# LinXueyuanStdio/LaTeX_OCR

Measured on NVIDIA H100. Metric: formula-images/sec (train step, 128x512 px, seq<=150), higher is better.
Workload: dtype bf16

## Files before the change

### latex_ocr_b200/csrc/lo_common.cuh

```cuda
#pragma once
#include <cuda_runtime.h>
#include <cuda_bf16.h>
#include <stdint.h>
#include <stdio.h>
#include <string.h>

#include "../../include/latex_ocr_b200.h"

typedef __nv_bfloat16 bf16;

namespace lo {

extern char g_err[512];
extern int64_t g_launches;

inline int fail(int code, const char* fmt, const char* a = "", long b = 0, long c = 0) {
  snprintf(g_err, sizeof(g_err), fmt, a, b, c);
  return code;
}

#define LO_CHECK_ARG(cond, what)                                                        \
  do {                                                                                  \
    if (!(cond)) return lo::fail(LO_EINVAL, "%s: invalid argument: " what " (line %ld)", __func__, __LINE__); \
  } while (0)
// ... 189 lines not shown
int gemm_nn(const void* A, int dtA, int64_t lda, const void* B, int dtB, int64_t ldb, void* C, int dtC, int64_t ldc,
            int M, int N, int K, int accumulate, int impl, cudaStream_t st);
int colsum(const void* X, int dt, float* out, int M, int N, int64_t ld, int accumulate, cudaStream_t st);

struct AttFwdArgs {
  const void *att1, *enc;
  const float* att2; int64_t att2_stride;
  const float* wf;
  float* alpha; int64_t alpha_stride;
  float* ctx; float* gate_pre; int64_t gate_stride; float* gctx; bf16* gctx_bf;
  int B, R;
  void* work;
  int rows_per_img;
  int act;
  int a_ch;
  uint8_t* mask_out;
  int abi = 0;
};
struct AttBwdArgs {
  const void *att1, *enc;
  const float *att2, *gate; int64_t o1_stride;
  const float* wf; const float* alpha; int64_t alpha_stride;
  const float* ctx; const float* dgctx; int64_t dg_stride;
  const float* dreg; int64_t dreg_stride; const float* sreg; int64_t sreg_stride;
  float* de; float* datt2; float* dgp; int64_t dcat_stride; bf16* datt2_bf; bf16* dgp_bf; float* dctx_out;
  int B, R;
  void* work;
  float* dwf_part;
  int act;
  int a_ch;
  const uint8_t* mask_in;
  int abi = 0;
  void* datt1 = nullptr;
  int ordered_dwf = 0;
};
int attention_fwd_pipe(const AttFwdArgs& x, int dt, int C, cudaStream_t st);
int attention_bwd_pipe(const AttBwdArgs& x, int dt, int C, cudaStream_t st);
inline int64_t att_partials_offset(int B) { return B <= 1024 ? 4096 : ((int64_t)B * 4 + 255) / 256 * 256; }
struct AttRagged {
  const int32_t* reg_off;
  const int32_t* reg_off_host;
  void* map;
  int ctas;
};
int64_t attention_ragged_map_bytes(int B);
int attention_ragged_prepare(AttRagged& rg, int B, int rpi, cudaStream_t st);
int attention_fwd_ragged(const AttFwdArgs& x, const AttRagged& rg, int dt, int C, cudaStream_t st);

bool tc_available();
int tc_gemm_nt(const bf16* A, int64_t lda, const bf16* W, int64_t ldw, void* C, int dtC, int64_t ldc,
               int M, int N, int K, const float* bias, int accumulate, int relu, cudaStream_t st);
int tc_gemm_nt_ex(const bf16* A, int64_t lda, const bf16* W, int64_t ldw, void* C, int dtC, int64_t ldc, int M, int N, int K,
                  const float* bias, int accumulate, int relu, int splits, int atomic_acc, int small_n_tile, cudaStream_t st);
int skinny_gemm_nt(const bf16* A, int64_t lda, const bf16* W, int64_t ldw, float* C, int64_t ldc, int M, int N, int K, const float* bias,
                   int splits, int atomic_acc, cudaStream_t st);
int resident_ctas(const void* kernel, int threads, size_t smem);
int tc_gemm_tn(const bf16* A, int64_t lda, const bf16* B, int64_t ldb, float* C, int64_t ldc, int M, int N, int K, cudaStream_t st);
int tc_gemm_tn_batched(const bf16* A, int64_t sAk, int64_t sAb, const bf16* B, int64_t sBk, int64_t sBb, float* C, int64_t ldc,
                       int64_t sCb, int M, int N, int K, int batch, cudaStream_t st);
int tc_conv3x3_wgrad(const bf16* x, const bf16* dy, float* dw, int N, int H, int W, int Cin, int Cout, int pad, cudaStream_t st);
int tc_conv3x3(const bf16* x, const bf16* w, const float* bias, const bf16* mask, bf16* y,
               int N, int H, int W, int Cin, int Cout, int pad, int relu, cudaStream_t st);

}
```

### latex_ocr_b200/csrc/lo_decoder.cu

```cuda
#include "lo_common.cuh"
#include "lo_ptx.cuh"

namespace lo {

#define LO_ATT_THREADS 256
#define LO_ATT_WARPS 8
#define LO_ATT_MAXSPLIT 16

static inline int att_splits(int B) {
  int s = (444 + B - 1) / B;
  if (s < 1) s = 1;
  if (s > LO_ATT_MAXSPLIT) s = LO_ATT_MAXSPLIT;
  return s;
}

__device__ __forceinline__ float ldcg_f(const float* p) { return __ldcg(p); }

template <typename T, int NV>
__global__ void __launch_bounds__(LO_ATT_THREADS) attention_fwd_kernel(
    const T* __restrict__ att1, const T* __restrict__ enc, const float* __restrict__ att2, int64_t att2_stride,
    const float* __restrict__ wf, float* __restrict__ alpha, int64_t alpha_stride, float* __restrict__ ctx,
    float* __restrict__ gate_pre, int64_t gate_stride, float* __restrict__ gctx, bf16* __restrict__ gctx_bf, int R, int nsplit,
    int* __restrict__ counters, float* __restrict__ partials, int rpi) {
  constexpr int CH = NV * 256;
// ... 1112 lines not shown

__global__ void split_bf16_kernel(const float* __restrict__ x, bf16* __restrict__ hi, bf16* __restrict__ lo, int64_t n) {
  for (int64_t i = blockIdx.x * (int64_t)blockDim.x + threadIdx.x; i < n; i += (int64_t)gridDim.x * blockDim.x) {
    const float v = x[i];
    const bf16 h = __float2bfloat16_rn(v);
    hi[i] = h;
    lo[i] = __float2bfloat16_rn(v - __bfloat162float(h));
  }
}

static int forward_prologue(const lo_decoder_args* a, const Dims& d, cudaStream_t st) {
  const int dt = a->dt;
  const int rpi = a->rows_per_img > 1 ? a->rows_per_img : 1;
  const int enc_rows = a->reg_off_host ? a->reg_off_host[d.B / rpi] : (d.B / rpi) * d.R;
  LO_TRY(gemm_nt(a->enc, dt, d.C, a->w_enc_att, dt, d.C, a->att1, dt, d.A, enc_rows, d.A, d.C, a->b_enc_att, 0, 0, a->impl, st));
  const BfViews bv0 = bf_views(a, d);
  if (bv0.on && d.E % 64 == 0) {
    LO_TRY(tc_gemm_nt_ex((const bf16*)a->emb, d.E, (const bf16*)a->w_ih, d.E + d.C, a->ptab, LO_F32, d.G, d.V, d.G, d.E, a->b_ih, 0, 0, 1,
                         0, 0, st));
  } else {
    LO_TRY(gemm_nt(a->emb, dt, d.E, a->w_ih, dt, d.E + d.C, a->ptab, LO_F32, d.G, d.V, d.G, d.E, a->b_ih, 0, 0, LO_IMPL_SIMT, st));
  }
  {
    dim3 grid(cdiv(d.C, 256), d.B);
    if (a->reg_off)
      LO_DISPATCH_DT(dt, T, (mean_segments_kernel<T><<<grid, 256, 0, st>>>((const T*)a->enc, a->mean, a->reg_off, d.C, rpi)));
    else
      LO_DISPATCH_DT(dt, T, (mean_rows_kernel<T><<<grid, 256, 0, st>>>((const T*)a->enc, a->mean, d.R, d.C, rpi)));
    LO_LAUNCH_OK();
  }
  const size_t es = dt == LO_F32 ? 4 : 2;
  if (bv0.on && d.C % 64 == 0 && d.T >= 2) {
    bf16* mean_hi = bv0.gctx;
    bf16* mean_lo = bv0.gctx + (int64_t)d.B * d.C;
    split_bf16_kernel<<<cdiv((long)d.B * d.C, 256), 256, 0, st>>>(a->mean, mean_hi, mean_lo, (int64_t)d.B * d.C);
    LO_LAUNCH_OK();
    const bf16* w_h = (const bf16*)a->w_init;
    const bf16* w_c = w_h + (int64_t)d.D * d.C;
    LO_TRY(tc_gemm_nt_ex(mean_hi, d.C, w_h, d.C, a->hall, LO_F32, d.D, d.B, d.D, d.C, a->b_init, 0, 0, 1, 0, 1, st));
    LO_TRY(tc_gemm_nt_ex(mean_lo, d.C, w_h, d.C, a->hall, LO_F32, d.D, d.B, d.D, d.C, nullptr, 1, 0, 1, 0, 1, st));
    LO_TRY(tc_gemm_nt_ex(mean_hi, d.C, w_c, d.C, a->call, LO_F32, d.D, d.B, d.D, d.C, a->b_init + d.D, 0, 0, 1, 0, 1, st));
    LO_TRY(tc_gemm_nt_ex(mean_lo, d.C, w_c, d.C, a->call, LO_F32, d.D, d.B, d.D, d.C, nullptr, 1, 0, 1, 0, 1, st));
  } else {
    LO_TRY(gemm_nt(a->mean, LO_F32, d.C, a->w_init, dt, d.C, a->hall, LO_F32, d.D, d.B, d.D, d.C, a->b_init, 0, 0, LO_IMPL_SIMT, st));
    LO_TRY(gemm_nt(a->mean, LO_F32, d.C, (const char*)a->w_init + (size_t)d.D * d.C * es, dt, d.C, a->call, LO_F32, d.D, d.B,
                   d.D, d.C, a->b_init + d.D, 0, 0, LO_IMPL_SIMT, st));
  }
  const BfViews bv = bf_views(a, d);
  if (bv.on) LO_TRY(lo_cast(a->hall, LO_F32, bv.hall, LO_BF16, (int64_t)d.B * d.D, (void*)st));
  return LO_OK;
}

static int step_gemm_nt(bool tc, const float* A32, const bf16* Abf, int64_t lda, const void* W, int dtW, int64_t ldw, float* C,
                        int64_t ldc, int M, int N, int K, const float* bias, int acc, int splits, int atomic_acc, cudaStream_t st) {
  if (tc && g_opt_skinny_mma && M <= 64) return skinny_gemm_nt(Abf, lda, (const bf16*)W, ldw, C, ldc, M, N, K, bias, splits, atomic_acc, st);
  if (tc)
    return tc_gemm_nt_ex(Abf, lda, (const bf16*)W, ldw, C, LO_F32, ldc, M, N, K, bias, 0, 0, g_opt_det ? 1 : splits, atomic_acc, 1, st);
  return gemm_nt(A32, LO_F32, lda, W, dtW, ldw, C, LO_F32, ldc, M, N, K, bias, acc, 0, LO_IMPL_SIMT, st);
}

static int head_nt(const lo_decoder_args* a, bool tc, const float* h32, const bf16* hbf, int64_t ldh, float* logits, int64_t ldl, int M,
                   cudaStream_t st) {
  if (tc) return gemm_nt(hbf, LO_BF16, ldh, a->w_fc, LO_BF16, a->D, logits, LO_F32, ldl, M, a->V, a->D, a->b_fc, 0, 0, LO_IMPL_TC, st);
  return gemm_nt(h32, LO_F32, ldh, a->w_fc, a->dt, a->D, logits, LO_F32, ldl, M, a->V, a->D, a->b_fc, 0, 0, LO_IMPL_SIMT, st);
}

static int forward_step(const lo_decoder_args* a, const Dims& d, int t, int nrows, const AttRagged* rg, const int64_t* tok,
                        int64_t tok_stride, float* hd_t, int64_t hd_stride, const float* dmask_t, cudaStream_t st) {
  const int dt = a->dt;
  const bool sampling = a->ss_prob && hd_t;
  const size_t es = dt == LO_F32 ? 4 : 2;
  const int64_t cur = (int64_t)t * d.B, nxt = (int64_t)(t + 1) * d.B;
  float* o1 = a->out1 + cur * d.O1;
  const BfViews bv = bf_views(a, d);
  if (!(g_opt_dbg_skip & 4))
    LO_TRY(step_gemm_nt(bv.on, a->hall + cur * d.D, bv.on ? bv.hall + cur * d.D : nullptr, d.D, a->wcat1, dt, d.D, o1, d.O1, nrows,
                        d.O1, d.D, a->bcat1, 0, 1, 0, st));
  if (rg) {
    if (!(g_opt_dbg_skip & 2)) {
      AttFwdArgs x{a->att1, a->enc, o1, d.O1, a->w_full, a->alphas + t * d.R, (int64_t)d.T * d.R, a->ctx + cur * d.C, o1 + d.A,
                   d.O1, a->gctx + cur * d.C, bv.on ? bv.gctx + cur * d.C : nullptr, nrows, d.R, a->work, a->rows_per_img, 0, 0, nullptr, 0};
      LO_TRY(attention_fwd_ragged(x, *rg, dt, d.C, st));
    }
  } else if (!(g_opt_dbg_skip & 2))
  LO_TRY(attention_forward_launch(a->att1, a->enc, dt, o1, d.O1, a->w_full, a->alphas + t * d.R, (int64_t)d.T * d.R, a->ctx + cur * d.C,
                                  o1 + d.A, d.O1, a->gctx + cur * d.C, bv.on ? bv.gctx + cur * d.C : nullptr, nrows, d.R, d.C, a->work, st,
                                  a->rows_per_img, hd_t ? att_mask_at(a, t) : nullptr));
  if (g_opt_dbg_skip & 4) return LO_OK;
  LO_TRY(step_gemm_nt(bv.on, a->gctx + cur * d.C, bv.on ? bv.gctx + cur * d.C : nullptr, d.C, (const char*)a->w_ih + (size_t)d.E * es, dt,
                      d.E + d.C, a->gtmp, d.G, nrows, d.G, d.C, nullptr, 0, 1, 0, st));
  SsStep ss{};
  if (sampling) {
    ss.prev_logits = t > 0 ? a->logits + (int64_t)(t - 1) * d.Vl : nullptr;
    ss.lstride = (int64_t)d.T * d.Vl;
    ss.prob = a->ss_prob;
    ss.u = a->ss_u ? a->ss_u + t : nullptr;
    ss.coin_state = (const unsigned long long*)a->dropout_state;
    ss.ustride = d.T;
    ss.fed = a->fed + t;
    ss.hd_bf = bv.on ? bv.hd + t * d.D : nullptr;
  }
  auto launch_pw = [&](auto kernel, auto... extra) {
    return launch_pdl(kernel, dim3(cdiv((long)nrows * d.D, 256)), dim3(256), (size_t)0, st, (const float*)a->gtmp,
                      (const float*)a->ptab, tok, tok_stride, (const float*)(o1 + d.A + d.C), (int64_t)d.O1,
                      (const float*)(a->call + cur * d.D), a->gates + cur * d.G, a->call + nxt * d.D, a->hall + nxt * d.D,
                      bv.on ? bv.hall + nxt * d.D : (bf16*)nullptr, hd_t, hd_stride, dmask_t, nrows, d.D, d.V,
                      (const unsigned long long*)((hd_t && a->has_dropout == 2) ? a->dropout_state : nullptr), a->dropout_p, 0, t, ss,
                      extra...);
  };
  if (sampling && a->ss_temp) {
    const GumbelStep gs{a->ss_temp, a->ss_gu ? a->ss_gu + (int64_t)t * d.V : nullptr, (int64_t)d.T * d.V};
    LO_CUDA(launch_pw(lstm_pw_fwd_gumbel_kernel, gs));
  } else {
    LO_CUDA(launch_pw(sampling ? lstm_pw_fwd_kernel<true> : lstm_pw_fwd_kernel<false>));
  }
  LO_LAUNCH_OK();
  if (sampling) {
    LO_TRY(head_nt(a, bv.on, hd_t, ss.hd_bf, hd_stride, a->logits + (int64_t)t * d.Vl, (int64_t)d.T * d.Vl, nrows, st));
  }
  return LO_OK;
}

static int backward_step(const lo_decoder_args* a, const Dims& d, int t, int nrows, const float* dal, int64_t dal_b, int64_t dal_t,
                         cudaStream_t st) {
  const int dt = a->dt;
  const BfViews bv = bf_views(a, d);
  const int64_t cur = (int64_t)t * d.B, nxt = (int64_t)(t + 1) * d.B;
  float* dcat_t = a->dcat + cur * d.O1;
  bf16* dcat_bf_t = bv.on ? bv.dcat + cur * d.O1 : nullptr;
  const float* o1 = a->out1 + cur * d.O1;
  float* dxh = a->dxh;
  const float* dmul = (a->has_dropout == 1 && a->dropout_mask) ? a->dropout_mask + (int64_t)t * d.D : nullptr;
  if (!(g_opt_dbg_skip & 4))
    LO_CUDA(launch_pdl(lstm_pw_bwd_kernel, dim3(cdiv((long)nrows * d.D, 256)), dim3(256), (size_t)0, st,
                       (const float*)(a->dhd + (int64_t)t * d.D), (int64_t)d.T * d.D, dmul, (const float*)(dxh + d.C),
                       (int64_t)(d.C + d.D), a->dc, (const float*)(a->gates + cur * d.G), (const float*)(a->call + cur * d.D),
                       (const float*)(a->call + nxt * d.D), dcat_t + d.A + d.C, (int64_t)d.O1,
                       bv.on ? dcat_bf_t + d.A + d.C : (bf16*)nullptr, bv.on ? dxh : (float*)nullptr, d.C, nrows, d.D,
                       (const unsigned long long*)(a->has_dropout == 2 ? a->dropout_state : nullptr), a->dropout_p, 0, t));
  LO_LAUNCH_OK();
  if (!(g_opt_dbg_skip & 4))
    LO_TRY(step_gemm_nt(bv.on, dcat_t + d.A + d.C, bv.on ? dcat_bf_t + d.A + d.C : nullptr, d.O1, a->wbwd1, dt, d.G, dxh, d.C + d.D,
                        nrows, d.C + d.D, d.G, nullptr, 0, 4, 1, st));
  const float* alpha_t = a->alphas + t * d.R;
  const float* ctx_t = a->ctx + cur * d.C;
  const float* dal_t_ptr = dal + (int64_t)t * dal_t;
  const float* sreg_t = a->sreg + t;
  float* de_t = a->de + t * d.R;
  float* dctx_t = a->dctx + cur * d.C;
  if (g_opt_dbg_skip & 2) {
  } else if (g_opt_att_pipe) {
    AttBwdArgs x{a->att1, a->enc, o1, o1 + d.A, d.O1, a->w_full, alpha_t, (int64_t)d.T * d.R, ctx_t, dxh, d.C + d.D, dal_t_ptr, dal_b,
                 sreg_t, d.T, de_t, dcat_t, dcat_t + d.A, d.O1, dcat_bf_t, dcat_bf_t ? dcat_bf_t + d.A : nullptr, dctx_t, nrows, d.R,
                 a->work, a->dmean, 0, 0, att_mask_at(a, t)};
    x.ordered_dwf = g_opt_det;
    LO_TRY(attention_bwd_pipe(x, dt, d.C, st));
  } else {
    const int ns = att_splits(d.B);
    int* cnt_c = (int*)a->work;
    float* part_c = (float*)((char*)a->work + att_partials_offset(nrows));
    dim3 grid(ns, nrows);
#define LO_ATT_BWD(TY_, NV)                                                                                                       \
  attention_bwd_kernel<TY_, NV><<<grid, LO_ATT_THREADS, 0, st>>>(                                                                 \
      (const TY_*)a->att1, (const TY_*)a->enc, o1, o1 + d.A, d.O1, a->w_full, alpha_t, (int64_t)d.T * d.R, ctx_t, dxh, d.C + d.D,    \
      dal_t_ptr, dal_b, sreg_t, d.T, de_t, dcat_t, dcat_t + d.A, d.O1, dcat_bf_t, dcat_bf_t ? dcat_bf_t + d.A : nullptr, dctx_t, d.R, \
      ns, cnt_c, part_c)
    if (dt == LO_F32) {
      if (d.C == 256) LO_ATT_BWD(float, 1); else if (d.C == 512) LO_ATT_BWD(float, 2); else LO_ATT_BWD(float, 4);
    } else {
      if (d.C == 256) LO_ATT_BWD(bf16, 1); else if (d.C == 512) LO_ATT_BWD(bf16, 2); else LO_ATT_BWD(bf16, 4);
    }
#undef LO_ATT_BWD
    LO_LAUNCH_OK();
  }
  if (!(g_opt_dbg_skip & 4))
    LO_TRY(step_gemm_nt(bv.on, dcat_t, dcat_bf_t, d.O1, a->wbwd2, dt, d.A + d.C, dxh + d.C, d.C + d.D, nrows, d.D, d.A + d.C, nullptr, 1,
                        4, 1, st));
  return LO_OK;
}

static size_t beam_step_smem(int beam, int V, bool second) { return (size_t)beam * V * 4 * (second ? 2 : 1); }

struct BeamPenStep {
  const float* len_pen;
  const float* cov_term;
  const int32_t* len_in;
  int32_t* len_out;
  float* scores;
};

static int beam_select(const float* logits, int V, int beam, int n_img, int t, int max_steps, int64_t end_id, float* logp,
                       int32_t* finished, int64_t* ids, int64_t* parents, int32_t* fin_hist, int64_t* next_tok, int32_t* parent_rows,
                       bool div_on, float div_gamma, float div_prob, const float* div_u_t, const uint64_t* div_state,
                       const BeamPenStep& ps, cudaStream_t st) {
  static bool smem_attr = false;
  const size_t smem = beam_step_smem(beam, V, div_on || ps.len_in);
  if (!smem_attr && smem > 48 * 1024) {
    LO_CUDA(cudaFuncSetAttribute(beam_step_kernel, cudaFuncAttributeMaxDynamicSharedMemorySize, 200 * 1024));
    smem_attr = true;
  }
  beam_step_kernel<<<n_img, 256, smem, st>>>(logits, V, beam, t, end_id, logp, finished, ids, parents, fin_hist, next_tok, parent_rows,
                                             max_steps, div_on ? logf(div_gamma) : 0.f, div_on ? div_prob : 0.f, div_u_t,
                                             (const unsigned long long*)div_state, ps.len_pen, ps.cov_term, ps.len_in, ps.len_out,
                                             ps.scores);
  LO_LAUNCH_OK();
  return LO_OK;
}

template <bool VEC>
__global__ void __launch_bounds__(256) beam_backtrack_kernel(const int64_t* __restrict__ ids, const int64_t* __restrict__ parents,
                                                             int64_t ids_stride_steps, int beam, int n, const float* __restrict__ alphas,
                                                             int64_t alpha_row_stride, int R, const int32_t* __restrict__ reg_off,
                                                             int lineage, int64_t* __restrict__ ids_out, float* __restrict__ att_out) {
  extern __shared__ int32_t s_bt[];
  int32_t* s_slot = s_bt + n * beam;
  int32_t* s_row = s_slot + n;
  const int img = blockIdx.x / beam, s = blockIdx.x % beam, tid = threadIdx.x;
  const int64_t src0 = (int64_t)img * ids_stride_steps * beam;
  if (lineage) {
    for (int j = tid; j < n * beam; j += blockDim.x) {
      const int64_t p = parents[src0 + j];
      s_bt[j] = (p >= 0 && p < beam) ? (int32_t)p : 0;
    }
    __syncthreads();
    if (tid == 0) {
      int cur = s;
      for (int t = n - 1; t >= 0; t--) {
        s_slot[t] = cur;
        cur = s_bt[t * beam + cur];
        s_row[t] = cur;
// ... 659 lines not shown
```

### latex_ocr_b200/csrc/lo_skinny.cu

```cuda
#include "lo_common.cuh"
#include "lo_ptx.cuh"

namespace lo {

constexpr int SK_KC = 512;
constexpr int SK_NT = 16;
constexpr int SK_PITCH = SK_KC + 8;
constexpr int SK_SMEM = (64 + SK_NT) * SK_PITCH * 2;

__device__ __forceinline__ void cp_async16(void* dst, const void* src, bool valid) {
  const int sz = valid ? 16 : 0;
  asm volatile("cp.async.cg.shared.global [%0], [%1], 16, %2;" ::"r"(smem_u32(dst)), "l"(src), "r"(sz) : "memory");
}
__device__ __forceinline__ void ldmatrix_x4(uint32_t& r0, uint32_t& r1, uint32_t& r2, uint32_t& r3, const void* p) {
  asm volatile("ldmatrix.sync.aligned.m8n8.x4.shared.b16 {%0, %1, %2, %3}, [%4];"
               : "=r"(r0), "=r"(r1), "=r"(r2), "=r"(r3)
               : "r"(smem_u32(p)));
}
__device__ __forceinline__ void mma_bf16_16816(float* c, uint32_t a0, uint32_t a1, uint32_t a2, uint32_t a3, uint32_t b0, uint32_t b1) {
  asm volatile("mma.sync.aligned.m16n8k16.row.col.f32.bf16.bf16.f32 {%0, %1, %2, %3}, {%4, %5, %6, %7}, {%8, %9}, {%0, %1, %2, %3};"
               : "+f"(c[0]), "+f"(c[1]), "+f"(c[2]), "+f"(c[3])
               : "r"(a0), "r"(a1), "r"(a2), "r"(a3), "r"(b0), "r"(b1));
}

template <bool TMA>
__global__ void __launch_bounds__(128) skinny_mma_kernel(const bf16* __restrict__ A, int64_t lda, const bf16* __restrict__ W, int64_t ldw,
                                                          float* __restrict__ C, int64_t ldc, int M, int N, int K, int kc,
                                                          const float* __restrict__ bias, int mode) {
  A += (int64_t)blockIdx.z * 64 * lda;
  C += (int64_t)blockIdx.z * 64 * ldc;
  M = min(64, M - (int)blockIdx.z * 64);
  extern __shared__ __align__(16) uint8_t sk_smem[];
  bf16* sA = reinterpret_cast<bf16*>(sk_smem);
  bf16* sW = sA + 64 * SK_PITCH;
  const int n0 = blockIdx.x * SK_NT;
  const int k0 = blockIdx.y * kc;
  const int kn = min(kc, K - k0);
  const int tid = threadIdx.x, warp = tid >> 5, lane = tid & 31;
  const int cpr = kn / 8;
  float bpre[2][2];
#pragma unroll
  for (int j = 0; j < 2; j++) {
    const int n = n0 + j * 8 + 2 * (lane & 3);
    const bool has = bias && blockIdx.y == 0 && n < N;
    bpre[j][0] = has ? bias[n] : 0.f;
    bpre[j][1] = has ? bias[n + 1] : 0.f;
  }
  if constexpr (TMA) {
    uint64_t* bars = reinterpret_cast<uint64_t*>(sk_smem + SK_SMEM);
    if (tid == 0) {
      mbar_init(bars, 1);
      mbar_init(bars + 1, 1);
      fence_barrier_init();
    }
    __syncthreads();
    const uint32_t row_bytes = (uint32_t)kn * 2u;
    if (warp == 0) {
      const int wrows = min(SK_NT, N - n0);
      const uint64_t pol = l2_policy_evict_last();
      if (lane == 0) mbar_expect_tx(bars, (uint32_t)wrows * row_bytes);
      __syncwarp();
      if (lane < wrows) bulk_g2s(sW + lane * SK_PITCH, W + (int64_t)(n0 + lane) * ldw + k0, row_bytes, bars, pol);
    }
    for (int i = tid; i < (SK_NT - min(SK_NT, N - n0)) * cpr; i += 128)
      *reinterpret_cast<uint4*>(sW + (min(SK_NT, N - n0) + i / cpr) * SK_PITCH + (i % cpr) * 8) = make_uint4(0, 0, 0, 0);
    for (int i = tid; i < (64 - M) * cpr; i += 128)
      *reinterpret_cast<uint4*>(sA + (M + i / cpr) * SK_PITCH + (i % cpr) * 8) = make_uint4(0, 0, 0, 0);
    pdl_wait();
    pdl_trigger();
    if (warp == 0) {
      const uint64_t pol = l2_policy_evict_first();
      if (lane == 0) mbar_expect_tx(bars + 1, (uint32_t)M * row_bytes);
      __syncwarp();
      for (int r = lane; r < M; r += 32) bulk_g2s(sA + r * SK_PITCH, A + (int64_t)r * lda + k0, row_bytes, bars + 1, pol);
    }
    mbar_wait(bars, 0);
    mbar_wait(bars + 1, 0);
    __syncthreads();
  } else {
  for (int i = tid; i < SK_NT * cpr; i += 128) {
    const int r = i / cpr, c = i % cpr;
    cp_async16(sW + r * SK_PITCH + c * 8, W + (int64_t)min(n0 + r, N - 1) * ldw + k0 + c * 8, n0 + r < N);
  }
  pdl_wait();
  pdl_trigger();
  for (int i = tid; i < 64 * cpr; i += 128) {
    const int r = i / cpr, c = i % cpr;
    cp_async16(sA + r * SK_PITCH + c * 8, A + (int64_t)min(r, M - 1) * lda + k0 + c * 8, r < M);
  }
  asm volatile("cp.async.commit_group;\n\tcp.async.wait_group 0;" ::: "memory");
  __syncthreads();
  }
  float acc[2][4] = {{0.f, 0.f, 0.f, 0.f}, {0.f, 0.f, 0.f, 0.f}};
  float acd[2][4] = {{0.f, 0.f, 0.f, 0.f}, {0.f, 0.f, 0.f, 0.f}};
  const bf16* a_ptr = sA + (warp * 16 + (lane & 7) + ((lane >> 3) & 1) * 8) * SK_PITCH + (lane >> 4) * 8;
  const bf16* b_ptr = sW + ((lane & 7) + (lane >> 4) * 8) * SK_PITCH + ((lane >> 3) & 1) * 8;
  int k = 0;
#pragma unroll 4
  for (; k + 32 <= kn; k += 32) {
    uint32_t a0, a1, a2, a3, b0, b1, b2, b3, c0, c1, c2, c3, d0, d1, d2, d3;
    ldmatrix_x4(a0, a1, a2, a3, a_ptr + k);
    ldmatrix_x4(b0, b1, b2, b3, b_ptr + k);
    ldmatrix_x4(c0, c1, c2, c3, a_ptr + k + 16);
    ldmatrix_x4(d0, d1, d2, d3, b_ptr + k + 16);
    mma_bf16_16816(acc[0], a0, a1, a2, a3, b0, b1);
    mma_bf16_16816(acc[1], a0, a1, a2, a3, b2, b3);
    mma_bf16_16816(acd[0], c0, c1, c2, c3, d0, d1);
    mma_bf16_16816(acd[1], c0, c1, c2, c3, d2, d3);
  }
  if (k < kn) {
    uint32_t a0, a1, a2, a3, b0, b1, b2, b3;
    ldmatrix_x4(a0, a1, a2, a3, a_ptr + k);
    ldmatrix_x4(b0, b1, b2, b3, b_ptr + k);
    mma_bf16_16816(acc[0], a0, a1, a2, a3, b0, b1);
    mma_bf16_16816(acc[1], a0, a1, a2, a3, b2, b3);
  }
#pragma unroll
  for (int j = 0; j < 2; j++)
#pragma unroll
    for (int q = 0; q < 4; q++) acc[j][q] += acd[j][q] + bpre[j][q & 1];
  if (gridDim.y > 1 && mode != 1) {
    __syncthreads();
    float* part = reinterpret_cast<float*>(sk_smem);
#pragma unroll
    for (int i = 0; i < 8; i++) part[i * 128 + tid] = acc[i >> 2][i & 3];
    cl_sync();
    if (cl_rank() == 0) {
      float s[8];
      cl_sum_n<8>(part + tid, 128, s);
#pragma unroll
      for (int i = 0; i < 8; i++) acc[i >> 2][i & 3] = s[i];
    }
    cl_sync();
    if (cl_rank() != 0) return;
  }
  const int g = lane >> 2, t = lane & 3;
#pragma unroll
  for (int j = 0; j < 2; j++) {
    const int n = n0 + j * 8 + 2 * t;
    if (n >= N) continue;
#pragma unroll
    for (int h = 0; h < 2; h++) {
      const int r = warp * 16 + g + h * 8;
      if (r >= M) continue;
      float* o = C + (int64_t)r * ldc + n;
      float x = acc[j][2 * h], y = acc[j][2 * h + 1];
      if (mode == 1) {
        atomicAdd(o, x);
        atomicAdd(o + 1, y);
        continue;
      }
      if (mode == 2) { const float2 old = *reinterpret_cast<float2*>(o); x += old.x; y += old.y; }
      *reinterpret_cast<float2*>(o) = make_float2(x, y);
    }
  }
}

int skinny_gemm_nt(const bf16* A, int64_t lda, const bf16* W, int64_t ldw, float* C, int64_t ldc, int M, int N, int K, const float* bias,
                   int splits, int atomic_acc, cudaStream_t st) {
  LO_CHECK_ARG(M >= 1 && M <= 64 * 1024 && K % 16 == 0 && N % 2 == 0 && lda % 8 == 0 && ldw % 8 == 0 && ldc % 2 == 0, "K%16, ld%8");
  static bool attr = false;
  if (!attr) {
    LO_CUDA(cudaFuncSetAttribute(skinny_mma_kernel<false>, cudaFuncAttributeMaxDynamicSharedMemorySize, SK_SMEM));
    LO_CUDA(cudaFuncSetAttribute(skinny_mma_kernel<true>, cudaFuncAttributeMaxDynamicSharedMemorySize, SK_SMEM + 16));
    attr = true;
  }
  int ks = cdiv(K, SK_KC);
  if (splits > ks) ks = splits;
  int kc = cdiv(cdiv(K, ks), 16) * 16;
  if (kc > SK_KC) kc = SK_KC;
  ks = cdiv(K, kc);
  if (!g_opt_det || ks == 1) {
    const int mode = (ks > 1 || atomic_acc) ? 1 : 0;
    if (ks > 1 && !atomic_acc) LO_CUDA(cudaMemset2DAsync(C, (size_t)ldc * 4, 0, (size_t)N * 4, (size_t)M, st));
    const dim3 grid(cdiv(N, SK_NT), ks, cdiv(M, 64));
    if (g_opt_skinny_tma) {
      LO_CUDA(launch_pdl(skinny_mma_kernel<true>, grid, dim3(128), (size_t)SK_SMEM + 16, st, A, lda, W, ldw, C, ldc, M, N, K, kc, bias, mode));
    } else {
      LO_CUDA(launch_pdl(skinny_mma_kernel<false>, grid, dim3(128), (size_t)SK_SMEM, st, A, lda, W, ldw, C, ldc, M, N, K, kc, bias, mode));
    }
    LO_LAUNCH_OK();
    return LO_OK;
  }
  for (int k0 = 0; k0 < K; k0 += 8 * kc) {
    const int kg = K - k0 < 8 * kc ? K - k0 : 8 * kc, ng = cdiv(kg, kc);
    const int mode = (k0 > 0 || atomic_acc) ? 2 : 0;
    const float* bg = k0 == 0 ? bias : nullptr;
    const dim3 grid(cdiv(N, SK_NT), ng, cdiv(M, 64)), cl(1, ng, 1);
    if (g_opt_skinny_tma) {
      LO_CUDA(launch_cluster(skinny_mma_kernel<true>, grid, dim3(128), (size_t)SK_SMEM + 16, st, cl, true, A + k0, lda, W + k0, ldw, C, ldc, M,
                             N, kg, kc, bg, mode));
    } else {
      LO_CUDA(launch_cluster(skinny_mma_kernel<false>, grid, dim3(128), (size_t)SK_SMEM, st, cl, true, A + k0, lda, W + k0, ldw, C, ldc, M, N,
                             kg, kc, bg, mode));
    }
    LO_LAUNCH_OK();
  }
  return LO_OK;
}

}
```

Measured before the change: 2546.

## Compute independent recurrent-gradient product before PDL wait in skinny GEMM

The backward step's dh product (the part of dcat times wbwd1 that feeds the hidden-state gradient) depends only on data that is ready early. It is now split off and computed inside the next skinny GEMM launch, before that kernel's programmatic-dependent-launch wait. The earlier GEMM now produces only the C columns, and the fused kernel runs the extra product while the previous kernel is still finishing. This shortens the serial critical path of the recurrent backward loop, at the cost of more shared memory per CTA, a second template instantiation, and extra smem loads before the PDL wait.

```diff
diff --git a/latex_ocr_b200/csrc/lo_common.cuh b/latex_ocr_b200/csrc/lo_common.cuh
--- a/latex_ocr_b200/csrc/lo_common.cuh
+++ b/latex_ocr_b200/csrc/lo_common.cuh
@@ -265,8 +265,20 @@
                int M, int N, int K, const float* bias, int accumulate, int relu, cudaStream_t st);
 int tc_gemm_nt_ex(const bf16* A, int64_t lda, const bf16* W, int64_t ldw, void* C, int dtC, int64_t ldc, int M, int N, int K,
                   const float* bias, int accumulate, int relu, int splits, int atomic_acc, int small_n_tile, cudaStream_t st);
+struct SkinnyPre {
+  const bf16* A;
+  int64_t lda;
+  const bf16* W;
+  int64_t ldw;
+  float* C;
+  int64_t ldc;
+  int K;
+  const float* bias;
+  int splits, atomic_acc;
+};
+bool skinny_pre_fits(int K, int splits, int K2, int splits2);
 int skinny_gemm_nt(const bf16* A, int64_t lda, const bf16* W, int64_t ldw, float* C, int64_t ldc, int M, int N, int K, const float* bias,
-                   int splits, int atomic_acc, cudaStream_t st);
+                   int splits, int atomic_acc, cudaStream_t st, const SkinnyPre* pre = nullptr);
 int resident_ctas(const void* kernel, int threads, size_t smem);
 int tc_gemm_tn(const bf16* A, int64_t lda, const bf16* B, int64_t ldb, float* C, int64_t ldc, int M, int N, int K, cudaStream_t st);
 int tc_gemm_tn_batched(const bf16* A, int64_t sAk, int64_t sAb, const bf16* B, int64_t sBk, int64_t sBb, float* C, int64_t ldc,
diff --git a/latex_ocr_b200/csrc/lo_decoder.cu b/latex_ocr_b200/csrc/lo_decoder.cu
--- a/latex_ocr_b200/csrc/lo_decoder.cu
+++ b/latex_ocr_b200/csrc/lo_decoder.cu
@@ -1188,11 +1188,18 @@
 }
 
 static int step_gemm_nt(bool tc, const float* A32, const bf16* Abf, int64_t lda, const void* W, int dtW, int64_t ldw, float* C,
-                        int64_t ldc, int M, int N, int K, const float* bias, int acc, int splits, int atomic_acc, cudaStream_t st) {
-  if (tc && g_opt_skinny_mma && M <= 64) return skinny_gemm_nt(Abf, lda, (const bf16*)W, ldw, C, ldc, M, N, K, bias, splits, atomic_acc, st);
+                        int64_t ldc, int M, int N, int K, const float* bias, int acc, int splits, int atomic_acc, cudaStream_t st,
+                        const SkinnyPre* pre = nullptr) {
+  if (tc && g_opt_skinny_mma && M <= 64)
+    return skinny_gemm_nt(Abf, lda, (const bf16*)W, ldw, C, ldc, M, N, K, bias, splits, atomic_acc, st, pre);
+  LO_CHECK_ARG(!pre, "a second product needs the mma.sync kernel");
   if (tc)
     return tc_gemm_nt_ex(Abf, lda, (const bf16*)W, ldw, C, LO_F32, ldc, M, N, K, bias, 0, 0, g_opt_det ? 1 : splits, atomic_acc, 1, st);
   return gemm_nt(A32, LO_F32, lda, W, dtW, ldw, C, LO_F32, ldc, M, N, K, bias, acc, 0, LO_IMPL_SIMT, st);
+}
+
+static bool recurrent_prewait(bool tc, int M, int K, int splits, int K2, int splits2) {
+  return tc && g_opt_skinny_mma && M <= 64 && skinny_pre_fits(K, splits, K2, splits2);
 }
 
 static int head_nt(const lo_decoder_args* a, bool tc, const float* h32, const bf16* hbf, int64_t ldh, float* logits, int64_t ldl, int M,
@@ -1275,9 +1282,10 @@
                        bv.on ? dcat_bf_t + d.A + d.C : (bf16*)nullptr, bv.on ? dxh : (float*)nullptr, d.C, nrows, d.D,
                        (const unsigned long long*)(a->has_dropout == 2 ? a->dropout_state : nullptr), a->dropout_p, 0, t));
   LO_LAUNCH_OK();
+  const bool pre = recurrent_prewait(bv.on, nrows, d.A + d.C, 4, d.G, 4);
   if (!(g_opt_dbg_skip & 4))
     LO_TRY(step_gemm_nt(bv.on, dcat_t + d.A + d.C, bv.on ? dcat_bf_t + d.A + d.C : nullptr, d.O1, a->wbwd1, dt, d.G, dxh, d.C + d.D,
-                        nrows, d.C + d.D, d.G, nullptr, 0, 4, 1, st));
+                        nrows, pre ? d.C : d.C + d.D, d.G, nullptr, 0, 4, 1, st));
   const float* alpha_t = a->alphas + t * d.R;
   const float* ctx_t = a->ctx + cur * d.C;
   const float* dal_t_ptr = dal + (int64_t)t * dal_t;
@@ -1309,9 +1317,11 @@
 #undef LO_ATT_BWD
     LO_LAUNCH_OK();
   }
+  const SkinnyPre dh{pre ? dcat_bf_t + d.A + d.C : nullptr, d.O1, (const bf16*)a->wbwd1 + (int64_t)d.C * d.G, d.G, dxh + d.C, d.C + d.D,
+                     d.G, nullptr, 4, 1};
   if (!(g_opt_dbg_skip & 4))
     LO_TRY(step_gemm_nt(bv.on, dcat_t, dcat_bf_t, d.O1, a->wbwd2, dt, d.A + d.C, dxh + d.C, d.C + d.D, nrows, d.D, d.A + d.C, nullptr, 1,
-                        4, 1, st));
+                        4, 1, st, pre ? &dh : nullptr));
   return LO_OK;
 }
 
diff --git a/latex_ocr_b200/csrc/lo_skinny.cu b/latex_ocr_b200/csrc/lo_skinny.cu
--- a/latex_ocr_b200/csrc/lo_skinny.cu
+++ b/latex_ocr_b200/csrc/lo_skinny.cu
@@ -7,6 +7,7 @@
 constexpr int SK_NT = 16;
 constexpr int SK_PITCH = SK_KC + 8;
 constexpr int SK_SMEM = (64 + SK_NT) * SK_PITCH * 2;
+constexpr int SK_SMEM_PRE = SK_SMEM + SK_NT * SK_PITCH * 2;
 
 __device__ __forceinline__ void cp_async16(void* dst, const void* src, bool valid) {
   const int sz = valid ? 16 : 0;
@@ -23,34 +24,144 @@
                : "r"(a0), "r"(a1), "r"(a2), "r"(a3), "r"(b0), "r"(b1));
 }
 
-template <bool TMA>
+struct SkPre {
+  const bf16* A;
+  int64_t lda;
+  const bf16* W;
+  int64_t ldw;
+  float* C;
+  int64_t ldc;
+  int K, kc;
+  const float* bias;
+  int mode;
+};
+
+__device__ __forceinline__ void sk_bias(const float* __restrict__ bias, int n0, int N, int lane, float (&bpre)[2][2]) {
+#pragma unroll
+  for (int j = 0; j < 2; j++) {
+    const int n = n0 + j * 8 + 2 * (lane & 3);
+    const bool has = bias && blockIdx.y == 0 && n < N;
+    bpre[j][0] = has ? bias[n] : 0.f;
+    bpre[j][1] = has ? bias[n + 1] : 0.f;
+  }
+}
+
+__device__ __forceinline__ void sk_mma(const bf16* sA, const bf16* sW, int kn, int warp, int lane, const float (&bpre)[2][2],
+                                       float (&acc)[2][4]) {
+  float acd[2][4] = {{0.f, 0.f, 0.f, 0.f}, {0.f, 0.f, 0.f, 0.f}};
+  const bf16* a_ptr = sA + (warp * 16 + (lane & 7) + ((lane >> 3) & 1) * 8) * SK_PITCH + (lane >> 4) * 8;
+  const bf16* b_ptr = sW + ((lane & 7) + (lane >> 4) * 8) * SK_PITCH + ((lane >> 3) & 1) * 8;
+  int k = 0;
+#pragma unroll 4
+  for (; k + 32 <= kn; k += 32) {
+    uint32_t a0, a1, a2, a3, b0, b1, b2, b3, c0, c1, c2, c3, d0, d1, d2, d3;
+    ldmatrix_x4(a0, a1, a2, a3, a_ptr + k);
+    ldmatrix_x4(b0, b1, b2, b3, b_ptr + k);
+    ldmatrix_x4(c0, c1, c2, c3, a_ptr + k + 16);
+    ldmatrix_x4(d0, d1, d2, d3, b_ptr + k + 16);
+    mma_bf16_16816(acc[0], a0, a1, a2, a3, b0, b1);
+    mma_bf16_16816(acc[1], a0, a1, a2, a3, b2, b3);
+    mma_bf16_16816(acd[0], c0, c1, c2, c3, d0, d1);
+    mma_bf16_16816(acd[1], c0, c1, c2, c3, d2, d3);
+  }
+  if (k < kn) {
+    uint32_t a0, a1, a2, a3, b0, b1, b2, b3;
+    ldmatrix_x4(a0, a1, a2, a3, a_ptr + k);
+    ldmatrix_x4(b0, b1, b2, b3, b_ptr + k);
+    mma_bf16_16816(acc[0], a0, a1, a2, a3, b0, b1);
+    mma_bf16_16816(acc[1], a0, a1, a2, a3, b2, b3);
+  }
+#pragma unroll
+  for (int j = 0; j < 2; j++)
+#pragma unroll
+    for (int q = 0; q < 4; q++) acc[j][q] += acd[j][q] + bpre[j][q & 1];
+}
+
+__device__ __forceinline__ void sk_cluster_sum(float* part, int tid, float (&acc)[2][4]) {
+  __syncthreads();
+#pragma unroll
+  for (int i = 0; i < 8; i++) part[i * 128 + tid] = acc[i >> 2][i & 3];
+  cl_sync();
+  if (cl_rank() == 0) {
+    float s[8];
+    cl_sum_n<8>(part + tid, 128, s);
+#pragma unroll
+    for (int i = 0; i < 8; i++) acc[i >> 2][i & 3] = s[i];
+  }
+  cl_sync();
+}
+
+__device__ __forceinline__ void sk_store(float* __restrict__ C, int64_t ldc, int M, int N, int n0, int warp, int lane, const float (&acc)[2][4],
+                                         int mode) {
+  const int g = lane >> 2, t = lane & 3;
+#pragma unroll
+  for (int j = 0; j < 2; j++) {
+    const int n = n0 + j * 8 + 2 * t;
+    if (n >= N) continue;
+#pragma unroll
+    for (int h = 0; h < 2; h++) {
+      const int r = warp * 16 + g + h * 8;
+      if (r >= M) continue;
+      float* o = C + (int64_t)r * ldc + n;
+      float x = acc[j][2 * h], y = acc[j][2 * h + 1];
+      if (mode == 1) {
+        atomicAdd(o, x);
+        atomicAdd(o + 1, y);
+        continue;
+      }
+      if (mode == 2) { const float2 old = *reinterpret_cast<float2*>(o); x += old.x; y += old.y; }
+      *reinterpret_cast<float2*>(o) = make_float2(x, y);
+    }
+  }
+}
+
+__device__ __forceinline__ void sk_pre_product(const SkPre& pre, const bf16* sA, bf16* sW2, float* C2, int M, int N, int n0, int kn2,
+                                               int tid, int warp, int lane, const float (&b2)[2][2]) {
+  float acc2[2][4] = {{0.f, 0.f, 0.f, 0.f}, {0.f, 0.f, 0.f, 0.f}};
+  sk_mma(sA, sW2, kn2, warp, lane, b2, acc2);
+  if (gridDim.y > 1 && pre.mode != 1) {
+    sk_cluster_sum(reinterpret_cast<float*>(sW2), tid, acc2);
+    if (cl_rank() == 0) sk_store(C2, pre.ldc, M, N, n0, warp, lane, acc2, pre.mode);
+  } else {
+    __syncthreads();
+    sk_store(C2, pre.ldc, M, N, n0, warp, lane, acc2, pre.mode);
+  }
+}
+
+template <bool TMA, bool PRE>
 __global__ void __launch_bounds__(128) skinny_mma_kernel(const bf16* __restrict__ A, int64_t lda, const bf16* __restrict__ W, int64_t ldw,
                                                           float* __restrict__ C, int64_t ldc, int M, int N, int K, int kc,
-                                                          const float* __restrict__ bias, int mode) {
+                                                          const float* __restrict__ bias, int mode, SkPre pre) {
   A += (int64_t)blockIdx.z * 64 * lda;
   C += (int64_t)blockIdx.z * 64 * ldc;
   M = min(64, M - (int)blockIdx.z * 64);
   extern __shared__ __align__(16) uint8_t sk_smem[];
   bf16* sA = reinterpret_cast<bf16*>(sk_smem);
   bf16* sW = sA + 64 * SK_PITCH;
+  bf16* sW2 = sW + SK_NT * SK_PITCH;
   const int n0 = blockIdx.x * SK_NT;
   const int k0 = blockIdx.y * kc;
   const int kn = min(kc, K - k0);
   const int tid = threadIdx.x, warp = tid >> 5, lane = tid & 31;
   const int cpr = kn / 8;
   float bpre[2][2];
-#pragma unroll
-  for (int j = 0; j < 2; j++) {
-    const int n = n0 + j * 8 + 2 * (lane & 3);
-    const bool has = bias && blockIdx.y == 0 && n < N;
-    bpre[j][0] = has ? bias[n] : 0.f;
-    bpre[j][1] = has ? bias[n + 1] : 0.f;
-  }
+  sk_bias(bias, n0, N, lane, bpre);
+  const int k02 = PRE ? blockIdx.y * pre.kc : 0;
+  const int kn2 = PRE ? min(pre.kc, pre.K - k02) : 0;
+  const int cpr2 = kn2 / 8;
+  const bf16* A2 = PRE ? pre.A + (int64_t)blockIdx.z * 64 * pre.lda : nullptr;
+  float* C2 = PRE ? pre.C + (int64_t)blockIdx.z * 64 * pre.ldc : nullptr;
+  float b2[2][2];
+  if constexpr (PRE) sk_bias(pre.bias, n0, N, lane, b2);
   if constexpr (TMA) {
-    uint64_t* bars = reinterpret_cast<uint64_t*>(sk_smem + SK_SMEM);
+    uint64_t* bars = reinterpret_cast<uint64_t*>(sk_smem + (PRE ? SK_SMEM_PRE : SK_SMEM));
     if (tid == 0) {
       mbar_init(bars, 1);
       mbar_init(bars + 1, 1);
+      if constexpr (PRE) {
+        mbar_init(bars + 2, 1);
+        mbar_init(bars + 3, 1);
+      }
       fence_barrier_init();
     }
     __syncthreads();
@@ -61,11 +172,31 @@
       if (lane == 0) mbar_expect_tx(bars, (uint32_t)wrows * row_bytes);
       __syncwarp();
       if (lane < wrows) bulk_g2s(sW + lane * SK_PITCH, W + (int64_t)(n0 + lane) * ldw + k0, row_bytes, bars, pol);
+      if constexpr (PRE) {
+        const uint32_t row_bytes2 = (uint32_t)kn2 * 2u;
+        if (lane == 0) {
+          mbar_expect_tx(bars + 2, (uint32_t)wrows * row_bytes2);
+          mbar_expect_tx(bars + 3, (uint32_t)M * row_bytes2);
+        }
+        __syncwarp();
+        if (lane < wrows) bulk_g2s(sW2 + lane * SK_PITCH, pre.W + (int64_t)(n0 + lane) * pre.ldw + k02, row_bytes2, bars + 2, pol);
+        const uint64_t pol_a = l2_policy_evict_first();
+        for (int r = lane; r < M; r += 32) bulk_g2s(sA + r * SK_PITCH, A2 + (int64_t)r * pre.lda + k02, row_bytes2, bars + 3, pol_a);
+      }
     }
     for (int i = tid; i < (SK_NT - min(SK_NT, N - n0)) * cpr; i += 128)
       *reinterpret_cast<uint4*>(sW + (min(SK_NT, N - n0) + i / cpr) * SK_PITCH + (i % cpr) * 8) = make_uint4(0, 0, 0, 0);
-    for (int i = tid; i < (64 - M) * cpr; i += 128)
-      *reinterpret_cast<uint4*>(sA + (M + i / cpr) * SK_PITCH + (i % cpr) * 8) = make_uint4(0, 0, 0, 0);
+    const int cpz = PRE ? max(cpr, cpr2) : cpr;
+    for (int i = tid; i < (64 - M) * cpz; i += 128)
+      *reinterpret_cast<uint4*>(sA + (M + i / cpz) * SK_PITCH + (i % cpz) * 8) = make_uint4(0, 0, 0, 0);
+    if constexpr (PRE) {
+      for (int i = tid; i < (SK_NT - min(SK_NT, N - n0)) * cpr2; i += 128)
+        *reinterpret_cast<uint4*>(sW2 + (min(SK_NT, N - n0) + i / cpr2) * SK_PITCH + (i % cpr2) * 8) = make_uint4(0, 0, 0, 0);
+      mbar_wait(bars + 2, 0);
+      mbar_wait(bars + 3, 0);
+      __syncthreads();
+      sk_pre_product(pre, sA, sW2, C2, M, N, n0, kn2, tid, warp, lane, b2);
+    }
     pdl_wait();
     pdl_trigger();
     if (warp == 0) {
@@ -81,6 +212,19 @@
   for (int i = tid; i < SK_NT * cpr; i += 128) {
     const int r = i / cpr, c = i % cpr;
     cp_async16(sW + r * SK_PITCH + c * 8, W + (int64_t)min(n0 + r, N - 1) * ldw + k0 + c * 8, n0 + r < N);
+  }
+  if constexpr (PRE) {
+    for (int i = tid; i < SK_NT * cpr2; i += 128) {
+      const int r = i / cpr2, c = i % cpr2;
+      cp_async16(sW2 + r * SK_PITCH + c * 8, pre.W + (int64_t)min(n0 + r, N - 1) * pre.ldw + k02 + c * 8, n0 + r < N);
+    }
+    for (int i = tid; i < 64 * cpr2; i += 128) {
+      const int r = i / cpr2, c = i % cpr2;
+      cp_async16(sA + r * SK_PITCH + c * 8, A2 + (int64_t)min(r, M - 1) * pre.lda + k02 + c * 8, r < M);
+    }
+    asm volatile("cp.async.commit_group;\n\tcp.async.wait_group 0;" ::: "memory");
+    __syncthreads();
+    sk_pre_product(pre, sA, sW2, C2, M, N, n0, kn2, tid, warp, lane, b2);
   }
   pdl_wait();
   pdl_trigger();
@@ -120,18 +264,7 @@
 #pragma unroll
     for (int q = 0; q < 4; q++) acc[j][q] += acd[j][q] + bpre[j][q & 1];
   if (gridDim.y > 1 && mode != 1) {
-    __syncthreads();
-    float* part = reinterpret_cast<float*>(sk_smem);
-#pragma unroll
-    for (int i = 0; i < 8; i++) part[i * 128 + tid] = acc[i >> 2][i & 3];
-    cl_sync();
-    if (cl_rank() == 0) {
-      float s[8];
-      cl_sum_n<8>(part + tid, 128, s);
-#pragma unroll
-      for (int i = 0; i < 8; i++) acc[i >> 2][i & 3] = s[i];
-    }
-    cl_sync();
+    sk_cluster_sum(reinterpret_cast<float*>(sk_smem), tid, acc);
     if (cl_rank() != 0) return;
   }
   const int g = lane >> 2, t = lane & 3;
@@ -156,44 +289,65 @@
   }
 }
 
+static int sk_slices(int K, int splits, int* kc) {
+  int ks = cdiv(K, SK_KC);
+  if (splits > ks) ks = splits;
+  *kc = cdiv(cdiv(K, ks), 16) * 16;
+  if (*kc > SK_KC) *kc = SK_KC;
+  return cdiv(K, *kc);
+}
+
+bool skinny_pre_fits(int K, int splits, int K2, int splits2) {
+  int kc, kc2;
+  const int ks = sk_slices(K, splits, &kc);
+  return ks == sk_slices(K2, splits2, &kc2) && ks <= 8;
+}
+
 int skinny_gemm_nt(const bf16* A, int64_t lda, const bf16* W, int64_t ldw, float* C, int64_t ldc, int M, int N, int K, const float* bias,
-                   int splits, int atomic_acc, cudaStream_t st) {
+                   int splits, int atomic_acc, cudaStream_t st, const SkinnyPre* pre) {
   LO_CHECK_ARG(M >= 1 && M <= 64 * 1024 && K % 16 == 0 && N % 2 == 0 && lda % 8 == 0 && ldw % 8 == 0 && ldc % 2 == 0, "K%16, ld%8");
+  LO_CHECK_ARG(!pre || (skinny_pre_fits(K, splits, pre->K, pre->splits) && pre->K % 16 == 0 && pre->lda % 8 == 0 && pre->ldw % 8 == 0 &&
+                        pre->ldc % 2 == 0), "second product: K slices, K%16, ld%8");
   static bool attr = false;
   if (!attr) {
-    LO_CUDA(cudaFuncSetAttribute(skinny_mma_kernel<false>, cudaFuncAttributeMaxDynamicSharedMemorySize, SK_SMEM));
-    LO_CUDA(cudaFuncSetAttribute(skinny_mma_kernel<true>, cudaFuncAttributeMaxDynamicSharedMemorySize, SK_SMEM + 16));
+    LO_CUDA(cudaFuncSetAttribute(skinny_mma_kernel<false, false>, cudaFuncAttributeMaxDynamicSharedMemorySize, SK_SMEM));
+    LO_CUDA(cudaFuncSetAttribute(skinny_mma_kernel<true, false>, cudaFuncAttributeMaxDynamicSharedMemorySize, SK_SMEM + 16));
+    LO_CUDA(cudaFuncSetAttribute(skinny_mma_kernel<false, true>, cudaFuncAttributeMaxDynamicSharedMemorySize, SK_SMEM_PRE));
+    LO_CUDA(cudaFuncSetAttribute(skinny_mma_kernel<true, true>, cudaFuncAttributeMaxDynamicSharedMemorySize, SK_SMEM_PRE + 32));
     attr = true;
   }
-  int ks = cdiv(K, SK_KC);
-  if (splits > ks) ks = splits;
-  int kc = cdiv(cdiv(K, ks), 16) * 16;
-  if (kc > SK_KC) kc = SK_KC;
-  ks = cdiv(K, kc);
+  int kc;
+  const int ks = sk_slices(K, splits, &kc);
+  SkPre p2{};
+  if (pre) {
+    p2 = SkPre{pre->A, pre->lda, pre->W, pre->ldw, pre->C, pre->ldc, pre->K, 0, pre->bias, 0};
+    sk_slices(pre->K, pre->splits, &p2.kc);
+  }
+  auto launch = [&](dim3 grid, bool cluster, const bf16* Ag, const bf16* Wg, int Kg, const float* bg, int mg) {
+    const size_t smem = pre ? (size_t)SK_SMEM_PRE + (g_opt_skinny_tma ? 32 : 0) : (size_t)SK_SMEM + (g_opt_skinny_tma ? 16 : 0);
+    auto kern = pre ? (g_opt_skinny_tma ? skinny_mma_kernel<true, true> : skinny_mma_kernel<false, true>)
+                    : (g_opt_skinny_tma ? skinny_mma_kernel<true, false> : skinny_mma_kernel<false, false>);
+    if (cluster)
+      return launch_cluster(kern, grid, dim3(128), smem, st, dim3(1, grid.y, 1), true, Ag, lda, Wg, ldw, C, ldc, M, N, Kg, kc, bg, mg, p2);
+    return launch_pdl(kern, grid, dim3(128), smem, st, Ag, lda, Wg, ldw, C, ldc, M, N, Kg, kc, bg, mg, p2);
+  };
   if (!g_opt_det || ks == 1) {
     const int mode = (ks > 1 || atomic_acc) ? 1 : 0;
     if (ks > 1 && !atomic_acc) LO_CUDA(cudaMemset2DAsync(C, (size_t)ldc * 4, 0, (size_t)N * 4, (size_t)M, st));
-    const dim3 grid(cdiv(N, SK_NT), ks, cdiv(M, 64));
-    if (g_opt_skinny_tma) {
-      LO_CUDA(launch_pdl(skinny_mma_kernel<true>, grid, dim3(128), (size_t)SK_SMEM + 16, st, A, lda, W, ldw, C, ldc, M, N, K, kc, bias, mode));
-    } else {
-      LO_CUDA(launch_pdl(skinny_mma_kernel<false>, grid, dim3(128), (size_t)SK_SMEM, st, A, lda, W, ldw, C, ldc, M, N, K, kc, bias, mode));
-    }
+    if (pre) {
+      p2.mode = (ks > 1 || pre->atomic_acc) ? 1 : 0;
+      if (ks > 1 && !pre->atomic_acc) LO_CUDA(cudaMemset2DAsync(pre->C, (size_t)pre->ldc * 4, 0, (size_t)N * 4, (size_t)M, st));
+    }
+    LO_CUDA(launch(dim3(cdiv(N, SK_NT), ks, cdiv(M, 64)), false, A, W, K, bias, mode));
     LO_LAUNCH_OK();
     return LO_OK;
   }
+  p2.mode = pre && pre->atomic_acc ? 2 : 0;
   for (int k0 = 0; k0 < K; k0 += 8 * kc) {
     const int kg = K - k0 < 8 * kc ? K - k0 : 8 * kc, ng = cdiv(kg, kc);
     const int mode = (k0 > 0 || atomic_acc) ? 2 : 0;
     const float* bg = k0 == 0 ? bias : nullptr;
-    const dim3 grid(cdiv(N, SK_NT), ng, cdiv(M, 64)), cl(1, ng, 1);
-    if (g_opt_skinny_tma) {
-      LO_CUDA(launch_cluster(skinny_mma_kernel<true>, grid, dim3(128), (size_t)SK_SMEM + 16, st, cl, true, A + k0, lda, W + k0, ldw, C, ldc, M,
-                             N, kg, kc, bg, mode));
-    } else {
-      LO_CUDA(launch_cluster(skinny_mma_kernel<false>, grid, dim3(128), (size_t)SK_SMEM, st, cl, true, A + k0, lda, W + k0, ldw, C, ldc, M, N,
-                             kg, kc, bg, mode));
-    }
+    LO_CUDA(launch(dim3(cdiv(N, SK_NT), ng, cdiv(M, 64)), true, A + k0, W + k0, kg, bg, mode));
     LO_LAUNCH_OK();
   }
   return LO_OK;
```

Result: no change. 2568, median of 6 (+0.9%).

## Retile skinny GEMM to 16-row M tile with warps split across N

Applied to the files above, without the earlier changes.

Changes the skinny GEMM block tile from 64 rows of A by 16 weight rows to 16 rows of A by 64 weight rows. Each warp now covers a different 16-column slice of N and shares the same A tile, instead of each warp covering a different 16-row slice of M. For small M (decode-like shapes), this avoids zero-padding A up to 64 rows and cuts the number of blocks along N, so each weight row is streamed once per 16 A rows. The cost is that weight reads are repeated for every 16-row M tile when M is large, and grid occupancy changes.

```diff
diff --git a/latex_ocr_b200/csrc/lo_skinny.cu b/latex_ocr_b200/csrc/lo_skinny.cu
--- a/latex_ocr_b200/csrc/lo_skinny.cu
+++ b/latex_ocr_b200/csrc/lo_skinny.cu
@@ -4,9 +4,10 @@
 namespace lo {
 
 constexpr int SK_KC = 512;
-constexpr int SK_NT = 16;
+constexpr int SK_MT = 16;
+constexpr int SK_NT = 64;
 constexpr int SK_PITCH = SK_KC + 8;
-constexpr int SK_SMEM = (64 + SK_NT) * SK_PITCH * 2;
+constexpr int SK_SMEM = (SK_MT + SK_NT) * SK_PITCH * 2;
 
 __device__ __forceinline__ void cp_async16(void* dst, const void* src, bool valid) {
   const int sz = valid ? 16 : 0;
@@ -27,21 +28,23 @@
 __global__ void __launch_bounds__(128) skinny_mma_kernel(const bf16* __restrict__ A, int64_t lda, const bf16* __restrict__ W, int64_t ldw,
                                                           float* __restrict__ C, int64_t ldc, int M, int N, int K, int kc,
                                                           const float* __restrict__ bias, int mode) {
-  A += (int64_t)blockIdx.z * 64 * lda;
-  C += (int64_t)blockIdx.z * 64 * ldc;
-  M = min(64, M - (int)blockIdx.z * 64);
+  A += (int64_t)blockIdx.z * SK_MT * lda;
+  C += (int64_t)blockIdx.z * SK_MT * ldc;
+  M = min(SK_MT, M - (int)blockIdx.z * SK_MT);
   extern __shared__ __align__(16) uint8_t sk_smem[];
   bf16* sA = reinterpret_cast<bf16*>(sk_smem);
-  bf16* sW = sA + 64 * SK_PITCH;
+  bf16* sW = sA + SK_MT * SK_PITCH;
   const int n0 = blockIdx.x * SK_NT;
+  const int wrows = min(SK_NT, N - n0);
   const int k0 = blockIdx.y * kc;
   const int kn = min(kc, K - k0);
   const int tid = threadIdx.x, warp = tid >> 5, lane = tid & 31;
   const int cpr = kn / 8;
+  const int nw = n0 + warp * 16;
   float bpre[2][2];
 #pragma unroll
   for (int j = 0; j < 2; j++) {
-    const int n = n0 + j * 8 + 2 * (lane & 3);
+    const int n = nw + j * 8 + 2 * (lane & 3);
     const bool has = bias && blockIdx.y == 0 && n < N;
     bpre[j][0] = has ? bias[n] : 0.f;
     bpre[j][1] = has ? bias[n + 1] : 0.f;
@@ -56,15 +59,14 @@
     __syncthreads();
     const uint32_t row_bytes = (uint32_t)kn * 2u;
     if (warp == 0) {
-      const int wrows = min(SK_NT, N - n0);
       const uint64_t pol = l2_policy_evict_last();
       if (lane == 0) mbar_expect_tx(bars, (uint32_t)wrows * row_bytes);
       __syncwarp();
-      if (lane < wrows) bulk_g2s(sW + lane * SK_PITCH, W + (int64_t)(n0 + lane) * ldw + k0, row_bytes, bars, pol);
-    }
-    for (int i = tid; i < (SK_NT - min(SK_NT, N - n0)) * cpr; i += 128)
-      *reinterpret_cast<uint4*>(sW + (min(SK_NT, N - n0) + i / cpr) * SK_PITCH + (i % cpr) * 8) = make_uint4(0, 0, 0, 0);
-    for (int i = tid; i < (64 - M) * cpr; i += 128)
+      for (int r = lane; r < wrows; r += 32) bulk_g2s(sW + r * SK_PITCH, W + (int64_t)(n0 + r) * ldw + k0, row_bytes, bars, pol);
+    }
+    for (int i = tid; i < (SK_NT - wrows) * cpr; i += 128)
+      *reinterpret_cast<uint4*>(sW + (wrows + i / cpr) * SK_PITCH + (i % cpr) * 8) = make_uint4(0, 0, 0, 0);
+    for (int i = tid; i < (SK_MT - M) * cpr; i += 128)
       *reinterpret_cast<uint4*>(sA + (M + i / cpr) * SK_PITCH + (i % cpr) * 8) = make_uint4(0, 0, 0, 0);
     pdl_wait();
     pdl_trigger();
@@ -72,7 +74,7 @@
       const uint64_t pol = l2_policy_evict_first();
       if (lane == 0) mbar_expect_tx(bars + 1, (uint32_t)M * row_bytes);
       __syncwarp();
-      for (int r = lane; r < M; r += 32) bulk_g2s(sA + r * SK_PITCH, A + (int64_t)r * lda + k0, row_bytes, bars + 1, pol);
+      if (lane < M) bulk_g2s(sA + lane * SK_PITCH, A + (int64_t)lane * lda + k0, row_bytes, bars + 1, pol);
     }
     mbar_wait(bars, 0);
     mbar_wait(bars + 1, 0);
@@ -84,7 +86,7 @@
   }
   pdl_wait();
   pdl_trigger();
-  for (int i = tid; i < 64 * cpr; i += 128) {
+  for (int i = tid; i < SK_MT * cpr; i += 128) {
     const int r = i / cpr, c = i % cpr;
     cp_async16(sA + r * SK_PITCH + c * 8, A + (int64_t)min(r, M - 1) * lda + k0 + c * 8, r < M);
   }
@@ -93,8 +95,8 @@
   }
   float acc[2][4] = {{0.f, 0.f, 0.f, 0.f}, {0.f, 0.f, 0.f, 0.f}};
   float acd[2][4] = {{0.f, 0.f, 0.f, 0.f}, {0.f, 0.f, 0.f, 0.f}};
-  const bf16* a_ptr = sA + (warp * 16 + (lane & 7) + ((lane >> 3) & 1) * 8) * SK_PITCH + (lane >> 4) * 8;
-  const bf16* b_ptr = sW + ((lane & 7) + (lane >> 4) * 8) * SK_PITCH + ((lane >> 3) & 1) * 8;
+  const bf16* a_ptr = sA + ((lane & 7) + ((lane >> 3) & 1) * 8) * SK_PITCH + (lane >> 4) * 8;
+  const bf16* b_ptr = sW + (warp * 16 + (lane & 7) + (lane >> 4) * 8) * SK_PITCH + ((lane >> 3) & 1) * 8;
   int k = 0;
 #pragma unroll 4
   for (; k + 32 <= kn; k += 32) {
@@ -137,11 +139,11 @@
   const int g = lane >> 2, t = lane & 3;
 #pragma unroll
   for (int j = 0; j < 2; j++) {
-    const int n = n0 + j * 8 + 2 * t;
+    const int n = nw + j * 8 + 2 * t;
     if (n >= N) continue;
 #pragma unroll
     for (int h = 0; h < 2; h++) {
-      const int r = warp * 16 + g + h * 8;
+      const int r = g + h * 8;
       if (r >= M) continue;
       float* o = C + (int64_t)r * ldc + n;
       float x = acc[j][2 * h], y = acc[j][2 * h + 1];
@@ -173,7 +175,7 @@
   if (!g_opt_det || ks == 1) {
     const int mode = (ks > 1 || atomic_acc) ? 1 : 0;
     if (ks > 1 && !atomic_acc) LO_CUDA(cudaMemset2DAsync(C, (size_t)ldc * 4, 0, (size_t)N * 4, (size_t)M, st));
-    const dim3 grid(cdiv(N, SK_NT), ks, cdiv(M, 64));
+    const dim3 grid(cdiv(N, SK_NT), ks, cdiv(M, SK_MT));
     if (g_opt_skinny_tma) {
       LO_CUDA(launch_pdl(skinny_mma_kernel<true>, grid, dim3(128), (size_t)SK_SMEM + 16, st, A, lda, W, ldw, C, ldc, M, N, K, kc, bias, mode));
     } else {
@@ -186,7 +188,7 @@
     const int kg = K - k0 < 8 * kc ? K - k0 : 8 * kc, ng = cdiv(kg, kc);
     const int mode = (k0 > 0 || atomic_acc) ? 2 : 0;
     const float* bg = k0 == 0 ? bias : nullptr;
-    const dim3 grid(cdiv(N, SK_NT), ng, cdiv(M, 64)), cl(1, ng, 1);
+    const dim3 grid(cdiv(N, SK_NT), ng, cdiv(M, SK_MT)), cl(1, ng, 1);
     if (g_opt_skinny_tma) {
       LO_CUDA(launch_cluster(skinny_mma_kernel<true>, grid, dim3(128), (size_t)SK_SMEM + 16, st, cl, true, A + k0, lda, W + k0, ldw, C, ldc, M,
                              N, kg, kc, bg, mode));
```

Result: faster. 2549 before, 2606 after, median of 6 (+2.2%).
